# neofytr/LLMTokenizer

Measured on AMD Instinct MI355X. Metric: corpus MB/s per merge iter (train), 1 GiB synthetic corpus, higher is better.
Workload: dtype u32

## Files before the change

llmtokenizer_amd/csrc/batch.hip:

```cpp
#pragma once
#include "engine_common.h"

namespace bpeamd {

static_assert(TOPK == 64, "a wave holds a list, one entry per lane");
static_assert(BRB == 2 * (1024 / 64), "the select's 16 waves merge two partial lists each");
#ifndef BPE_SU
#define BPE_SU 1
#endif
#ifndef BPE_FORM_PRINT
#define BPE_FORM_PRINT 0
#endif
#ifndef BPE_RU
#define BPE_RU 4
#endif
#ifndef BPE_AU
#define BPE_AU 1
#endif
constexpr uint32_t AU = BPE_AU;
constexpr uint32_t SU = BPE_SU;
#ifndef BPE_RUN_THREAD_PAIRS
#define BPE_RUN_THREAD_PAIRS 16
#endif
constexpr uint32_t RUN_THREAD_PAIRS = BPE_RUN_THREAD_PAIRS, RUN_Q = 256;
#ifndef BPE_RUN_BLOCK_Q
#define BPE_RUN_BLOCK_Q 2
#endif
constexpr uint32_t RUN_BLOCK_Q = BPE_RUN_BLOCK_Q;
#ifndef BPE_RUN_BU
#define BPE_RUN_BU 2
#endif
constexpr uint32_t RUN_BU = BPE_RUN_BU;
#ifndef BPE_FR
#define BPE_FR (BPE_BK > 63 ? 3 : 4)
#endif
// ... 1048 lines not shown
            s = (s + 1) & (RH - 1);
        }
    }
    __device__ inline uint32_t member(uint32_t a, uint32_t b) const {
        const unsigned long long key = (((unsigned long long)a << 32) | b) + 1ull;
        uint32_t s = rp_hash(a, b);
        for (;;) {
            const unsigned long long v = pk[s];
            if (v == key) return pm[s];
            if (v == 0ull) return BK;
            s = (s + 1) & (RP - 1);
        }
    }
};

__device__ inline void vadd_b(uint32_t (*s)[DENSE], const Eng *E, uint32_t m, int v, uint32_t x, uint32_t *gcnt) {
    if (x < DENSE) {
        atomicAdd(&s[v][x], 1u);
        return;
    }
    const uint64_t base = ((uint64_t)m * 4 + v) * E->bvs;
    const uint32_t old = atomicAdd(&E->bvec[base + (x - DENSE)], 1u);
    if (old == 0) {
        const uint32_t p = atomicAdd(&E->bvnl[m * 4 + v], 1u);
        E->bvlist[base + p] = x;
    }
    if (v == V_DL || v == V_DR) atomicAdd(&gcnt[v], 1u);
}

__device__ inline void vadd_g(const Eng *E, uint32_t m, int v, uint32_t x, uint32_t cnt) {
    if (!cnt) return;
    if (x < DENSE) {
        atomicAdd(&E->bvecd[((uint64_t)m * BREPL * 4 + v) * DENSE + x], cnt);
        return;
    }
    const uint64_t base = ((uint64_t)m * 4 + v) * E->bvs;
    if (atomicAdd(&E->bvec[base + (x - DENSE)], cnt) == 0) {
        const uint32_t p = atomicAdd(&E->bvnl[m * 4 + v], 1u);
        E->bvlist[base + p] = x;
    }
}

__device__ inline void xadd(const Eng *E, uint32_t *xo, uint32_t Wx, uint32_t m, int v, uint32_t x) {
    if (x < Wx) {
        atomicAdd(&xo[2 + v * Wx + x], 1u);
        return;
    }
    const uint64_t base = ((uint64_t)m * 4 + v) * E->bvs;
    if (atomicAdd(&E->bvec[base + (x - DENSE)], 1u) == 0) {
        const uint32_t p = atomicAdd(&E->bvnl[m * 4 + v], 1u);
        E->bvlist[base + p] = x;
    }
}

struct BHalo {
    uint32_t HL[3], HR[3], hlr[BK], myi[BK];
};

template <bool SH>
__device__ inline uint32_t tok_at_b(const uint32_t *__restrict__ tok, const BHalo &H, int64_t p, int64_t n) {
    if (p < 0) return SH && p >= -3 ? get3(H.HL, (uint32_t)(-1 - p)) : HOLE;
    if (p >= n) return SH && p - n < 3 ? get3(H.HR, (uint32_t)(p - n)) : HOLE;
    return tok[p];
}

template <bool SH>
__device__ inline uint32_t cover_of(const uint32_t *__restrict__ tok, const RoleTab &rt, const BHalo &H, uint32_t p,
                                    int64_t ps, int64_t n) {
    if (!(rt.get(p) >> 31)) return BK;
    const int64_t pps = v_left<SH>(tok, ps);
    const uint32_t pp = tok_at_b<SH>(tok, H, pps, n);
    const uint32_t mm = rt.member(pp, p);
    if (mm >= BK || pp != p) return mm;
    uint32_t L;
    if (SH && ps < 0) {
        L = H.hlr[mm];
    } else {
        L = 1;
        int64_t x = v_left<SH>(tok, ps);
        for (; x >= 0 && tok[x] == p; x = v_left<SH>(tok, x)) L++;
        if (SH && x < 0) L += H.hlr[mm];
    }
    return (L & 1) ? BK : mm;
}

template <bool SH>
__device__ inline uint32_t starts_of(const uint32_t *__restrict__ tok, const RoleTab &rt, const BHalo &H, uint32_t q,
                                     int64_t kq, int64_t n) {
    const uint32_t lq = rt.get(q) & 0x7FFFFFFFu;
    if (!lq) return BK;
    const int64_t kn = v_right(kq, lq, n);
    return rt.member(q, tok_at_b<SH>(tok, H, kn, n));
}

enum : uint32_t { GRF_LGO = 1, GRF_LEND = 2, GRF_IGO = 3, GRF_IEND = 4 };
__device__ void bscan_long_runs(const Eng *__restrict__ E, Bat *__restrict__ B, const uint32_t *__restrict__ tok,
                                const RoleTab &rt, const BHalo &H, int64_t n, uint32_t z0, uint32_t sgen) {
    const uint32_t lane = threadIdx.x & 63;
    const uint32_t ng = uni(min(aload(&B->gr_n), GRUN));
    const uint64_t stride = gr_stride(E->n0), maxch = stride - 1;
    auto flag_of = [&](uint32_t st) { return (sgen << 3) | st; };
    for (uint32_t gi = 0; gi < ng; gi++) {
        uint32_t ok = 1;
        if (lane == 0) {
            const unsigned long long t0 = wall_clock64();
            while (__hip_atomic_load(&B->gr_ready[gi], __ATOMIC_ACQUIRE, __HIP_MEMORY_SCOPE_AGENT) != sgen) {
                if (wall_clock64() - t0 > E->gr_wait) {
                    ok = 0;
                    B->ra_err = 11;
                    atomicAdd(&B->gr_tready, 1u);
                    break;
// ... 135 lines not shown
                vadd_g(E, mg, V_DR, ag, nint_dr);
                vadd_g(E, mg, V_IR, zg, nint_ir);
                if (npairs) atomicAdd(&B->bound[mg], npairs);
                atomicAdd(&B->nchunks, 1ull);
            }
#pragma unroll
            for (uint32_t bb = 0; bb < NBK; bb++) {
                unsigned long long tm = tadj.w[bb];
                for (int o = 32; o > 0; o >>= 1) tm |= __shfl_xor(tm, o);
                if (lane == 0 && tm) atomicOr(&B->adj[mg][bb], tm);
            }
        }
    }
}

template <bool SH>
__global__ __launch_bounds__(SCAN_T) void k_bscan(const Eng *__restrict__ E, const Ctl *__restrict__ C) {
    if (C->stop) return;
    Bat *B = E->bat;
    const uint32_t bi = bat_idx(E);
    ts_mark(E, bi, BT_SCAN_IN, true);
    if (threadIdx.x == 0) atomicMax(&B->sc_in, ~wall_clock64());
    __shared__ uint32_t s[4][DENSE];
    __shared__ uint32_t list[SCAN_T * SU * FR];
    __shared__ uint16_t ltag[SCAN_T * SU * FR];
    __shared__ uint32_t lcount, gbase, list_n, covc, sm, sk, sz0, bRs;
    __shared__ uint32_t lr_n, lr_brk, lr_pos[RUN_Q];
    __shared__ unsigned long long badj[NBK];
    __shared__ uint32_t gcnt[2];
    __shared__ uint32_t sa[BK], sb[BK];
    __shared__ RoleTab rt;
    __shared__ BHalo H;
    __shared__ uint32_t wmx[2][16];
    const uint32_t tid = threadIdx.x;
    const uint32_t sgen = ((uint32_t)(B->nbatch + B->nretry) & 0x0FFFFFFFu) + 1u;
    if (tid == 0) {
        sm = BK;
        covc = lcount = bRs = 0;
// ... 41 lines not shown
    }
    const uint32_t a = sa[m], b = sb[m], z = z0 + m;
    const uint32_t la = E->tlen[a], lb = E->tlen[b];
    const uint32_t mode = B->mode[m], off = B->off[m], len = B->len[m];
    const uint32_t bid = blockIdx.x - B->blk0[m], nblk = B->blk0[m + 1] - B->blk0[m];
    const uint32_t sbase = B->sbase[m];
    uint32_t *occz = E->ids_out + sbase;
    uint16_t *tagz = E->btag + sbase;
    const uint32_t sslice = B->sbase[m + 1] - sbase;
#define STG(IDX, WHERE) if ((IDX) >= sslice) { B->ra_err = 12; } else
    uint32_t *Rm = &B->R[m];
    const int64_t n = (int64_t)E->n0;
    const uint32_t *__restrict__ tok = E->tok;
    const uint32_t want = mode == 2 ? a : b;
    const uint32_t lim = min(DENSE, z0 + k);
    for (uint32_t v = 0; v < 4; v++)
        for (uint32_t x = tid; x < lim; x += SCAN_T) s[v][x] = 0;
    __syncthreads();
    auto tok_at = [&](int64_t p) -> uint32_t { return tok_at_b<SH>(tok, H, p, n); };

    if (a != b) {
        static_assert(SU == 1 && BPE_WFLUSH, "the wave-driven candidate loop: one entry per lane per round");
        const uint32_t stride = nblk * SCAN_T;
        const uint32_t lane = tid & 63, wbase = (tid >> 6) * 64 * FR;
        uint32_t wcnt = 0, wocc = 0;
        uint32_t nent[SU];
        uint16_t ntg[SU];
        uint32_t eS = bid * SCAN_T + (tid & ~63u);
        auto load1 = [&](uint32_t s0, uint32_t &en, uint16_t &tg) {
            const uint32_t e = s0 + lane;
            en = 0;
            tg = 0xFFFFu;
            if (e < len) {
                en = mode == 0 ? E->plist[off + e] : E->occ[off + e];
                if (mode) tg = E->occnb[off + e];
            }
        };
        uint32_t pent = 0;
        uint16_t ptg = 0xFFFFu;
        auto advance = [&]() {
            eS += stride;
            if (SCAN_PD > 1) {
                nent[0] = pent;
                ntg[0] = ptg;
                if (eS + stride < len) load1(eS + stride, pent, ptg);
            } else if (eS < len) {
                load1(eS, nent[0], ntg[0]);
            }
        };
        auto flush = [&]() {
            __builtin_amdgcn_fence(__ATOMIC_RELEASE, "wavefront");
            __builtin_amdgcn_wave_barrier();
            uint32_t g = 0;
            if (lane == 0 && wcnt) g = atomicAdd(Rm, wcnt);
            g = __shfl(g, 0);
            for (uint32_t q = lane; q < wcnt; q += 64) {
                STG(g + q, "wflush") {
                occz[g + q] = list[wbase + q];
                tagz[g + q] = ltag[wbase + q];
                }
            }
            wocc += wcnt;
            wcnt = 0;
            __builtin_amdgcn_wave_barrier();
        };
        const bool cmp = mode != 0 && E->scan_compact != 0;
        const uint32_t tsh = mode == 2 ? 8u : 0u;
        uint32_t qpos = 0, qn = 0;
        load1(eS, nent[0], ntg[0]);
        if (SCAN_PD > 1) load1(eS + stride, pent, ptg);
        for (;;) {
            uint32_t ent[SU];
            uint16_t etg[SU];
            bool val[SU];
            if (!cmp) {
                if (eS >= len) break;
                val[0] = eS + lane < len;
                ent[0] = nent[0];
                etg[0] = ntg[0];
                advance();
            } else {
                while (eS < len) {
                    const bool pass = eS + lane < len && tag_ok(((uint32_t)ntg[0] >> tsh) & 0xFFu, want);
                    const unsigned long long M = __ballot(pass);
                    const uint32_t np = (uint32_t)__popcll(M);
                    if (qn + np > 64) break;
                    const uint32_t r = lane - qn;
                    const bool mine = lane >= qn && r < np;
                    const uint32_t pv = (uint32_t)__shfl((int)nent[0], (int)(mine ? kth_bit(M, r) : lane));
                    if (mine) qpos = pv;
                    qn += np;
                    advance();
                }
                if (qn == 0) break;
                val[0] = lane < qn;
                ent[0] = qpos;
                etg[0] = 0xFFFFu;
                qn = 0;
            }
            int64_t ii[SU], jj[SU];
            TokWin W[SU];
#pragma unroll
            for (uint32_t u = 0; u < SU; u++) {
                if (mode == 2) {
                    val[u] = val[u] && tag_ok(etg[u] >> 8, want);
                    jj[u] = ent[u];
                    ii[u] = 0;
                    if (val[u]) W[u] = tok_window(tok, jj[u]);
                } else {
                    val[u] = val[u] && (mode == 0 || tag_ok(etg[u] & 0xFFu, want));
                    ii[u] = ent[u];
                    jj[u] = ii[u] + la;
                    if (val[u]) W[u] = tok_window(tok, ii[u]);
                }
            }
            bool ok[SU];
            uint32_t tl[SU], tr[SU];
#pragma unroll
            for (uint32_t u = 0; u < SU; u++) {
                ok[u] = false;
                tl[u] = tr[u] = HOLE;
                if (!val[u]) continue;
                const int64_t j = jj[u];
                if (mode == 2) {
                    const uint32_t wl = j > 0 ? W[u].at(j - 1) : HOLE;
                    const int64_t i = j > 0 ? start_of_end<SH>(wl, j - 1) : -1;
                    ii[u] = i;
                    if (W[u].at(j) != b || i < 0) continue;
                    const uint32_t ti = W[u].has(i) ? W[u].at(i) : tok[i];
                    tl[u] = i > 0 ? (W[u].has(i - 1) ? W[u].at(i - 1) : tok[i - 1]) : HOLE;
                    const int64_t kk = j + lb;
                    tr[u] = kk < n ? (W[u].has(kk) ? W[u].at(kk) : tok[kk]) : HOLE;
                    ok[u] = ti == a;
                } else {
                    const int64_t i = ii[u], kk = j + lb;
                    const uint32_t t1 = j >= n ? HOLE : W[u].has(j) ? W[u].at(j) : tok[j];
                    tl[u] = i > 0 ? W[u].at(i - 1) : HOLE;
                    tr[u] = kk >= n ? HOLE : W[u].has(kk) ? W[u].at(kk) : tok[kk];
                    ok[u] = W[u].at(i) == a && t1 == b && j < n;
                }
            }
            int64_t ps[SU];
            uint32_t pv[SU];
#pragma unroll
            for (uint32_t u = 0; u < SU; u++) {
                const int64_t i = ii[u];
                ps[u] = i <= 0 ? -1 : start_of_end<SH>(tl[u], i - 1);
                pv[u] = ok[u] ? ((i > 0 && is_id(tl[u])) ? tl[u] : tok_at(ps[u])) : HOLE;
            }
#pragma unroll
            for (uint32_t u = 0; u < SU; u++) {
                const int64_t i = ii[u], j = jj[u];
                uint32_t lfin = HOLE, rfin = HOLE;
                if (ok[u]) {
                    const uint32_t p = pv[u];
                    lfin = p;
                    if (p != HOLE) {
                        const uint32_t cv = cover_of<SH>(tok, rt, H, p, ps[u], n);
                        if (cv < BK) {
                            lfin = z0 + cv;
                            mk_set(tadj, cv);
                            atomicAdd(&covc, 1u);
                        } else {
                            vadd_b(s, E, m, V_DL, p, gcnt);
                            vadd_b(s, E, m, V_IL, p, gcnt);
                        }
                    }
                    const int64_t kq = v_right(j, lb, n);
                    const uint32_t q = kq < n ? tr[u] : tok_at(kq);
                    rfin = q;
                    if (q != HOLE) {
                        const uint32_t st = starts_of<SH>(tok, rt, H, q, kq, n);
                        if (st < BK) {
                            rfin = z0 + st;
                            mk_set(tadj, st);
                        }
                        vadd_b(s, E, m, V_DR, q, gcnt);
                        vadd_b(s, E, m, V_IR, rfin, gcnt);
                    }
                }
                const unsigned long long om = __ballot(ok[u]);
                if (ok[u]) {
                    const uint32_t slot = wbase + wcnt + (uint32_t)__popcll(om & ((1ull << lane) - 1ull));
                    list[slot] = (uint32_t)i;
                    ltag[slot] = nb_tag(lfin, rfin);
                }
                wcnt += (uint32_t)__popcll(om);
            }
            if (wcnt + 64 > 64 * FR) flush();
        }
        if (wcnt) flush();
        if (lane == 0 && wocc) atomicAdd(&bRs, wocc);
    } else {
        for (uint32_t e0 = bid * SCAN_T; e0 < len; e0 += nblk * SCAN_T) {
            const uint32_t e = e0 + tid;
            int64_t i = 0;
            bool ok = false;
            if (e >= len) {
            } else if (mode == 2) {
                const int64_t j = E->occ[off + e];
                if (tag_ok(E->occnb[off + e] >> 8, want) && tok[j] == b) {
                    i = v_left<SH>(tok, j);
                    ok = i >= 0 && tok[i] == a;
                }
// ... 23 lines not shown
                const uint32_t rq = nocc ? z : st < BK ? z0 + st : q;
                if (st < BK) mk_set(tadj, st);
                const uint32_t pfin = (mi > 0 || cont) ? z : (left ? p : cv < BK ? z0 + cv : HOLE);
                const uint32_t slot = atomicAdd(&lcount, 1u);
                if (slot < SCAN_T * SU) {
                    list[slot] = (uint32_t)pos;
                    ltag[slot] = nb_tag(pfin, rq);
                } else {
                    const uint32_t g = atomicAdd(Rm, 1u);
                    atomicAdd(&bRs, 1u);
                    STG(g, "tstraight") {
                    occz[g] = (uint32_t)pos;
                    tagz[g] = nb_tag(pfin, rq);
                    }
                }
                if (mi == 0 && left) {
                    vadd_b(s, E, m, V_DL, p, gcnt);
                    vadd_b(s, E, m, V_IL, p, gcnt);
                }
                if (q != HOLE) {
                    vadd_b(s, E, m, V_DR, q, gcnt);
                    vadd_b(s, E, m, V_IR, rq, gcnt);
                }
                if (!knext || kq >= n) break;
                if (mi + 1 >= RUN_THREAD_PAIRS && nocc) {
                    if (!SH && E->grflag && kq + (int64_t)GR_PROBE * la < n && tok[kq + (int64_t)GR_PROBE * la] == a) {
                        const uint32_t gi = atomicAdd(&B->gr_n, 1u);
                        if (gi < GRUN) {
                            B->gr_c[gi] = (uint32_t)kq;
                            B->gr_m[gi] = m;
                            atomicAdd(&B->gr_nreg, 1u);
                            __hip_atomic_store(&B->gr_ready[gi], sgen, __ATOMIC_RELEASE, __HIP_MEMORY_SCOPE_AGENT);
                            break;
                        }
// ... 104 lines not shown
                    });
                    const bool done = lr_brk < NS;
                    __syncthreads();
                    if (done) break;
                    c += (int64_t)NS * 64 * la;
                }
            }
        }
    }
    __syncthreads();
    if (!SH && E->grflag) bscan_long_runs(E, B, tok, rt, H, n, z0, sgen);
    ts_mark(E, bi, BT_SCAN_CAND, false, true);
    if (tid < SKMAX && tid < B->nsk && ((B->sk_cm[tid][m >> 6] >> (m & 63)) & 1ull)) {
        const uint32_t xs = B->sk_a[tid], ys = B->sk_b[tid];
        uint32_t d = 0;
        if (xs == b && ys < lim) d += s[V_DR][ys];
        if (ys == a && xs < lim) d += s[V_DL][xs];
        if (d) atomicAdd(SH ? &E->xbat[BK + tid] : &B->sdec[tid], d);
    }
    const uint32_t Wx = xbat_vw(z0 + k);
    uint32_t *xm = SH ? E->xbat + XBH + (uint64_t)m * xbat_member_words(Wx) : nullptr;
    if (SH && blockIdx.x == 0 && tid == 0) {
        uint32_t xlm = BK;
        const int64_t F1 = C->F1, L1 = C->L1;
        const uint32_t over = B->over;
        if (F1 < n) {
            const uint32_t tf = tok[F1], tl1 = tok[L1];
            for (uint32_t mm = 0; mm < k; mm++)
                if (H.HL[0] == sa[mm] && tf == sb[mm] && (sa[mm] != sb[mm] || (H.hlr[mm] & 1))) {
                    xlm = mm;
                    break;
                }
// ... 37 lines not shown
    if (k > 1) {
#pragma unroll
        for (uint32_t bb = 0; bb < NBK; bb++) {
            unsigned long long t = tadj.w[bb];
            for (int o = 32; o > 0; o >>= 1) t |= __shfl_xor(t, o);
            if ((tid & 63) == 0 && t) atomicOr(&badj[bb], t);
        }
        __syncthreads();
        if (tid < NBK && badj[tid]) atomicOr(&B->adj[m][tid], badj[tid]);
    }
    uint32_t *rep = SH ? xm + 2 : E->bvecd + (uint64_t)(m * BREPL + bid % BREPL) * 4 * DENSE;
    const uint32_t vstride = SH ? Wx : DENSE;
    uint32_t mxl = 0, mxr = 0;
    for (uint32_t v = 0; v < 4; v++)
        for (uint32_t x = tid; x < lim; x += SCAN_T) {
            const uint32_t c = s[v][x];
            if (c) atomicAdd(&rep[v * vstride + x], c);
            if (v == V_DL) mxl = max(mxl, c);
            if (v == V_DR) mxr = max(mxr, c);
        }
    if (SH && tid == 0 && bRs) atomicAdd(&xm[0], bRs);
    if (k > 1) {
        for (int o = 32; o > 0; o >>= 1) {
            mxl = max(mxl, (uint32_t)__shfl_xor(mxl, o));
            mxr = max(mxr, (uint32_t)__shfl_xor(mxr, o));
        }
        if ((tid & 63) == 0) {
            wmx[0][tid >> 6] = mxl;
            wmx[1][tid >> 6] = mxr;
        }
        __syncthreads();
        if (tid == 0) {
            uint32_t l = 0, r = 0;
            for (uint32_t q = 0; q < SCAN_T / 64; q++) {
                l = max(l, wmx[0][q]);
                r = max(r, wmx[1][q]);
            }
            atomicAdd(SH ? &xm[1] : &B->bound[m], max(l + gcnt[V_DL] + covc, r + gcnt[V_DR]));
        }
    }
    ts_mark(E, bi, BT_SCAN_OUT, false, true);
    asm volatile("s_waitcnt vmcnt(0)" ::: "memory");
    __syncthreads();
    if (tid == 0) atomicMax(&B->sc_out, wall_clock64());
}
template __global__ void k_bscan<false>(const Eng *, const Ctl *);
template __global__ void k_bscan<true>(const Eng *, const Ctl *);

constexpr uint32_t XSP_SHIFT = 23;
static_assert(4 * BK < (1u << (32 - XSP_SHIFT)), "member-vector index fits above the id");
__global__ __launch_bounds__(256) void k_bpack(const Eng *__restrict__ E, const Ctl *__restrict__ C) {
    if (C->stop) return;
    const Bat *B = E->bat;
    __shared__ uint32_t pre[BK * 4 + 1];
    __shared__ uint32_t written;
    const uint32_t k = B->k, tid = threadIdx.x, nmv = 4 * k;
    if (tid < 64) {
        constexpr uint32_t LP = 4 * NBK;
        uint32_t c[LP], sum = 0;
#pragma unroll
        for (uint32_t j = 0; j < LP; j++) {
            c[j] = LP * tid + j < nmv ? E->bvnl[LP * tid + j] : 0u;
// ... 652 lines not shown
```

llmtokenizer_amd/csrc/engine.hip:

```cpp
#include <hip/hip_runtime.h>
#include <fcntl.h>
#include <unistd.h>
#include <cerrno>

#include <algorithm>
#include <chrono>
#include <cstdio>
#include <cstdlib>
#include <cstring>
#include <string>
#include <thread>
#include <vector>
#include <unordered_map>

#include <rocprim/rocprim.hpp>

#include "../../include/bpe_gpu.h"
#include "kernels.hip"
#include "batch.hip"
#include "encode.hip"
#include "encode_win.hip"
#include "encode_docs.hip"
#include "split.hip"
#include "train_split.hip"
// ... 529 lines not shown
        if ((r = dalloc(c, &h.hotp_best, SPEC_RB))) return r;
        if ((r = dalloc(c, &h.hotp_key, SPEC_RB))) return r;
        if ((r = dalloc(c, &h.hotp_v2, SPEC_RB))) return r;
        if ((r = dalloc(c, &h.hotp_k2, SPEC_RB))) return r;
        if ((r = dalloc(c, &h.hotp_tie, SPEC_RB))) return r;
    }
    h.batch = getenv_int("BPE_BATCH", 1) && h.hot && h.vcap <= BATCH_VCAP_MAX && (!c->sharded || c->sbatch) &&
                      (c->sharded || c->fast || n0 >= TRACK_LIMIT)
                  ? 1
                  : 0;
    h.skip_on = (uint32_t)(getenv_int("BPE_SKIP", 1) != 0);
    if (h.skip_on && getenv_int("BPE_SKIP_TEST", 0)) h.skip_on = 2;
    h.skg_exp = (uint32_t)getenv_int("BPE_SKGATE", 2);
    h.scan_occd = (uint32_t)std::max(0, getenv_int("BPE_SCAN_OCCD", 6));
    h.scan_compact = (uint32_t)(getenv_int("BPE_SCAN_COMPACT", 1) != 0);
    {
        int nl = BK > 63 ? 2 : 1;
        if (getenv_int("BPE_LIST2", 0)) nl = std::max(nl, 2);
        nl = getenv_int("BPE_NLIST", nl);
        h.nlists = (uint32_t)std::max(1, std::min(nl, (int)NLIST));
    }
    h.tie_up = (uint32_t)(getenv_int("BPE_TIE_UP", 0) != 0);
    h.crate_pct = (uint32_t)std::max(100, getenv_int("BPE_CRATE_PCT", 200));
    h.lose_retry = (uint32_t)(getenv_int("BPE_TEST_LOSE_RETRY", 0) != 0);
    h.xbat = nullptr;
    h.xsp_out = h.xsp_in = nullptr;
    h.xsp_cap = 0;
    h.xsp_stride = 0;
    h.bat = nullptr;
    h.btag = nullptr;
// ... 216 lines not shown
        }
        return 0;
    }
    k_hot_collect<<<slots ? std::max<uint32_t>(1, std::min<uint32_t>(256, (ns + 255) / 256)) : 2048, 256, 0, c->st>>>(
        c->dE, c->dC, slots, ns);
    HIPCHK(hipGetLastError());
    return 0;
}

void launch_argmax_inputs(bpe_gpu_ctx *c) {
    launch_summaries(c);
    if (c->h.hot) k_hot_reduce<<<c->h.hot_parts, 1024, 0, c->st>>>(c->dE, c->dC);
}

void launch_batch(bpe_gpu_ctx *c) {
    k_bscan<false><<<BSB, SCAN_T, 0, c->st>>>(c->dE, c->dC);
    k_bapply<false><<<BAPPLY_B + BAPPLY_RA, 1024, 0, c->st>>>(c->dE, c->dC, BAPPLY_B);
    k_bsel<<<BRB + BAPPLY_A, 1024, 0, c->st>>>(c->dE, c->dC);
}

bool fused_graph(const bpe_gpu_ctx *c, bool tracked) { return c->h.spec_on && (!tracked || c->h.track_ub == 1); }

void launch_iteration(bpe_gpu_ctx *c, bool tracked) {
    if (fused_graph(c, tracked)) {
        const uint32_t trk = c->h.track_ub == 1 && !c->fast && c->n0 < TRACK_LIMIT ? 1 + (c->h.lcap ? LIGHT_B : 0) : 0;
        k_rescan_spec<<<SPEC_RB + SPEC_SB + trk, SCAN_T, 0, c->st>>>(c->dE, c->dC, SPEC_RB, trk);
        if (c->h.hcap / L1W > SELECT_L1_MAX && !c->h.hot) k_rescan2<<<RESCAN2_BLOCKS, 256, 0, c->st>>>(c->dE, c->dC);
        k_fused<<<1 + FUSED_A + FUSED_B, 1024, 0, c->st>>>(c->dE, c->dC, FUSED_A, nullptr);
        return;
    }
    k_scan<false><<<tracked ? TSCAN_BLOCKS : SCAN_BLOCKS, SCAN_T, 0, c->st>>>(c->dE, c->dC);
// ... 2840 lines not shown
```

llmtokenizer_amd/csrc/engine_common.h:

```cpp
#pragma once
#include <hip/hip_runtime.h>
#include <stddef.h>
#include <stdint.h>

namespace bpeamd {

constexpr uint32_t HOLE = 0xFFFFFFFFu;
constexpr uint32_t END_FLAG = 0x80000000u;
constexpr uint32_t MARKV = 0xFFFFFFFEu;
constexpr uint64_t END_MAX = 0x7FFFFFFDull;
__host__ __device__ inline bool is_id(uint32_t v) { return v < END_FLAG; }
__host__ __device__ inline uint32_t end_code(uint64_t d) { return END_FLAG | (uint32_t)d; }
#ifndef BPE_DENSE
#define BPE_DENSE 8192
#endif
constexpr uint32_t DENSE = BPE_DENSE;
#ifndef BPE_REPL
#define BPE_REPL 8
#endif
constexpr uint32_t REPL = BPE_REPL;
constexpr uint32_t NTHR = 16;
constexpr uint64_t CHUNK = 65536;
constexpr uint64_t DYN_LIMIT = CHUNK * NTHR;
constexpr uint64_t TRACK_LIMIT = 2 * DYN_LIMIT;
// ... 199 lines not shown
    uint32_t *erec;
    const uint32_t *enc_pairs;
    uint32_t n_enc;
    EncBatch *eb;
    uint32_t hot;
    uint32_t hot_parts;
    uint32_t hot_target;
    uint32_t relist_stale;
    uint32_t *hot_slot;
    uint32_t *hot_hist;
    unsigned long long *hotp_best, *hotp_key, *hotp_v2, *hotp_k2;
    uint32_t *hotp_tie;
    uint32_t batch;
    uint32_t skip_on;
    uint32_t scan_compact;
    uint32_t scan_occd;
    uint32_t skg_exp;
    uint32_t nlists;
    uint32_t tie_up;
    uint32_t crate_pct;
    uint32_t lose_retry;
    uint32_t bvs;
    Bat *bat;
    uint16_t *btag;
    uint32_t *bvecd;
    uint32_t *bvec;
    uint32_t *bvlist;
    uint32_t *bvnl;
    uint32_t *xbat;
    uint32_t *grflag;
// ... 203 lines not shown
```

llmtokenizer_amd/csrc/kernels.hip:

```cpp
#include "engine_common.h"
#include "p2p.hip"

namespace bpeamd {

__device__ inline uint32_t lane_id() { return __lane_id(); }

__device__ inline uint32_t aload(const uint32_t *p) {
    return __hip_atomic_load(p, __ATOMIC_RELAXED, __HIP_MEMORY_SCOPE_AGENT);
}
__device__ inline void astore(uint32_t *p, uint32_t v) {
    __hip_atomic_store(p, v, __ATOMIC_RELAXED, __HIP_MEMORY_SCOPE_AGENT);
}
__device__ inline unsigned long long aload64(const unsigned long long *p) {
    return __hip_atomic_load(p, __ATOMIC_RELAXED, __HIP_MEMORY_SCOPE_AGENT);
}

__device__ inline uint32_t wave_append(bool pred, uint32_t *counter) {
    unsigned long long m = __ballot(pred);
    if (m == 0) return 0;
    uint32_t lane = lane_id();
    uint32_t leader = __ffsll(m) - 1;
    uint32_t base = 0;
    if (lane == leader) base = atomicAdd(counter, (uint32_t)__popcll(m));
    base = __shfl(base, leader);
// ... 67 lines not shown
__device__ inline uint32_t id_at(const uint32_t *__restrict__ tok, HaloT &h, int64_t p, int64_t n) {
    if (p < 0) return SH && p >= -3 ? get3(h.get().HL, (uint32_t)(-1 - p)) : HOLE;
    if (p >= n) return SH && p - n < 3 ? get3(h.get().HR, (uint32_t)(p - n)) : HOLE;
    return tok[p];
}

template <bool SH = true>
__device__ inline int64_t start_of_end(uint32_t v, int64_t e) {
    if (is_id(v)) return e;
    if (SH && v == MARKV) return -1;
    const int64_t d = v & ~END_FLAG;
    if (!SH) return e - d;
    return d > e ? -1 : e - d;
}

template <bool SH = true>
__device__ inline int64_t v_left(const uint32_t *__restrict__ tok, int64_t p) {
    if (p <= 0) return p - 1;
    return start_of_end<SH>(tok[p - 1], p - 1);
}

__device__ inline int64_t v_right(int64_t p, uint32_t len, int64_t n) {
    if (p >= n) return p + 1;
    const int64_t q = p + len;
    return q >= n ? n : q;
}

constexpr uint32_t SCAN_T = 1024;

struct TokWin {
    uint4 w0, w1;
    int64_t base;
    __device__ inline bool has(int64_t x) const { return x >= base && x < base + 8; }
    __device__ inline uint32_t at(int64_t x) const {
        const uint32_t k = (uint32_t)(x - base);
        const uint4 w = k < 4 ? w0 : w1;
        const uint32_t r = k & 3;
        return r == 0 ? w.x : r == 1 ? w.y : r == 2 ? w.z : w.w;
    }
};

__device__ inline TokWin tok_window(const uint32_t *__restrict__ tok, int64_t i) {
    TokWin W;
    W.base = (i > 0 ? i - 1 : 0) & ~3ll;
    const uint4 *p = reinterpret_cast<const uint4 *>(tok + W.base);
    W.w0 = p[0];
    W.w1 = p[1];
    return W;
}

__device__ inline uint16_t nb_tag(uint32_t p, uint32_t q) {
    const uint32_t p8 = p == HOLE ? 0xFFu : (p & 0xFFu), q8 = q == HOLE ? 0xFFu : (q & 0xFFu);
    return (uint16_t)((p8 << 8) | q8);
}
__device__ inline bool tag_ok(uint32_t t8, uint32_t id) { return t8 == 0xFFu || t8 == (id & 0xFFu); }

__device__ inline void flush_list(uint32_t *list, uint16_t *ltag, uint32_t *lcount, uint32_t *gbase, uint32_t *R,
                                  uint32_t *occz, uint16_t *tagz, uint32_t *bcount) {
    __syncthreads();
    const uint32_t n = min(*lcount, SCAN_T);
    if (threadIdx.x == 0) {
        *gbase = n ? atomicAdd(R, n) : 0;
// ... 3185 lines not shown
```

llmtokenizer_amd/csrc/shard.hip:

```cpp
#include <dlfcn.h>
#include <rccl/rccl.h>


namespace {

struct RcclApi {
    void *lib = nullptr;
    ncclResult_t (*getUniqueId)(ncclUniqueId *) = nullptr;
    ncclResult_t (*commInitRank)(ncclComm_t *, int, ncclUniqueId, int) = nullptr;
    ncclResult_t (*allReduce)(const void *, void *, size_t, ncclDataType_t, ncclRedOp_t, ncclComm_t,
                              hipStream_t) = nullptr;
    ncclResult_t (*allGather)(const void *, void *, size_t, ncclDataType_t, ncclComm_t, hipStream_t) = nullptr;
    ncclResult_t (*commDestroy)(ncclComm_t) = nullptr;
    const char *(*errStr)(ncclResult_t) = nullptr;
};

int rccl_api(RcclApi **out) {
    static RcclApi api;
    if (!api.lib) {
        void *l = dlopen("librccl.so.1", RTLD_NOW | RTLD_GLOBAL);
        if (!l) l = dlopen("/opt/rocm/lib/librccl.so.1", RTLD_NOW | RTLD_GLOBAL);
        if (!l) return fail(BPE_GPU_ENODEV, "librccl.so.1 not loadable");
        api.getUniqueId = (decltype(api.getUniqueId))dlsym(l, "ncclGetUniqueId");
        api.commInitRank = (decltype(api.commInitRank))dlsym(l, "ncclCommInitRank");
// ... 192 lines not shown
    }
    if (g->rccl) {
        ncclResult_t e = g->rccl->allGather(c0->h.xsp_out, c0->h.xsp_in, stride, ncclUint32, g->comm, g->st);
        if (e != ncclSuccess) return rccl_fail(g->rccl, "ncclAllGather", e);
        return 0;
    }
    const uint32_t K = (uint32_t)g->cs.size();
    k_xspgather<<<K * K * 8, 256, 0, g->st>>>(g->d_ptrs + 4 * K, g->d_ptrs + 5 * K, K, stride);
    HIPCHK(hipGetLastError());
    return 0;
}

int launch_group_bstep(bpe_gpu_group *g) {
    int r;
    const bool sparse = g->cs[0]->h.xsp_out != nullptr;
    for (bpe_gpu_ctx *c : g->cs) k_bscan<true><<<BSB, SCAN_T, 0, g->st>>>(c->dE, c->dC);
    if (sparse)
        for (bpe_gpu_ctx *c : g->cs) k_bpack<<<64, 256, 0, g->st>>>(c->dE, c->dC);
    if ((r = ex_bsum(g))) return r;
    if (sparse && (r = ex_sparse(g))) return r;
    for (bpe_gpu_ctx *c : g->cs) k_bapply<true><<<BAPPLY_B + BAPPLY_RA, 1024, 0, g->st>>>(c->dE, c->dC, BAPPLY_B);
    for (bpe_gpu_ctx *c : g->cs) k_bsel<<<BRB + BAPPLY_A, 1024, 0, g->st>>>(c->dE, c->dC);
    HIPCHK(hipGetLastError());
    return ex_records(g, g->d_ptrs);
}

int group_bselect(bpe_gpu_group *g) {
    for (bpe_gpu_ctx *c : g->cs) k_bsel<<<BRB + BAPPLY_A, 1024, 0, g->st>>>(c->dE, c->dC);
    for (bpe_gpu_ctx *c : g->cs) k_edges<<<1, 256, 0, g->st>>>(c->dE, c->dC, 1);
    HIPCHK(hipGetLastError());
    return ex_records(g, g->d_ptrs);
// ... 997 lines not shown
```

Baseline: 114.9 million.

## Restructure bscan candidate loop to hoist dependent token loads and shrink shared histograms

Reworks the scan kernel's candidate loop so the dependent global token fetches (window, fringe tokens, left/right neighbour lookups, role-table flags) are issued in separate batched phases before use. The aim is more memory-level parallelism and fewer serialized load chains. Pointers are cast to the global address space so the compiler can emit plain global loads, and the shared histogram shrinks from four rows to three because the DL and IL rows are merged. An optional two-candidates-per-lane variant is added behind an env knob, but it is off by default. The cost is higher register pressure and some speculative loads for inactive lanes.

```diff
diff --git a/llmtokenizer_amd/csrc/batch.hip b/llmtokenizer_amd/csrc/batch.hip
--- a/llmtokenizer_amd/csrc/batch.hip
+++ b/llmtokenizer_amd/csrc/batch.hip
@@ -5,9 +5,6 @@
 
 static_assert(TOPK == 64, "a wave holds a list, one entry per lane");
 static_assert(BRB == 2 * (1024 / 64), "the select's 16 waves merge two partial lists each");
-#ifndef BPE_SU
-#define BPE_SU 1
-#endif
 #ifndef BPE_FORM_PRINT
 #define BPE_FORM_PRINT 0
 #endif
@@ -18,7 +15,6 @@
 #define BPE_AU 1
 #endif
 constexpr uint32_t AU = BPE_AU;
-constexpr uint32_t SU = BPE_SU;
 #ifndef BPE_RUN_THREAD_PAIRS
 #define BPE_RUN_THREAD_PAIRS 16
 #endif
@@ -1097,11 +1093,10 @@
     }
 };
 
-__device__ inline void vadd_b(uint32_t (*s)[DENSE], const Eng *E, uint32_t m, int v, uint32_t x, uint32_t *gcnt) {
-    if (x < DENSE) {
-        atomicAdd(&s[v][x], 1u);
-        return;
-    }
+enum { S_L = 0, S_DR = 1, S_IR = 2, S_N = 3 };
+__device__ constexpr int s_row(int v) { return v == V_DR ? S_DR : v == V_IR ? S_IR : S_L; }
+
+__device__ inline void vadd_bg(const Eng *E, uint32_t m, int v, uint32_t x, uint32_t *gcnt) {
     const uint64_t base = ((uint64_t)m * 4 + v) * E->bvs;
     const uint32_t old = atomicAdd(&E->bvec[base + (x - DENSE)], 1u);
     if (old == 0) {
@@ -1111,6 +1106,23 @@
     if (v == V_DL || v == V_DR) atomicAdd(&gcnt[v], 1u);
 }
 
+__device__ inline void vadd_b(uint32_t (*s)[DENSE], const Eng *E, uint32_t m, int v, uint32_t x, uint32_t *gcnt) {
+    if (x < DENSE) {
+        atomicAdd(&s[s_row(v)][x], 1u);
+        return;
+    }
+    vadd_bg(E, m, v, x, gcnt);
+}
+
+__device__ inline void vadd_bl(uint32_t (*s)[DENSE], const Eng *E, uint32_t m, uint32_t x, uint32_t *gcnt) {
+    if (x < DENSE) {
+        atomicAdd(&s[S_L][x], 1u);
+        return;
+    }
+    vadd_bg(E, m, V_DL, x, gcnt);
+    vadd_bg(E, m, V_IL, x, gcnt);
+}
+
 __device__ inline void vadd_g(const Eng *E, uint32_t m, int v, uint32_t x, uint32_t cnt) {
     if (!cnt) return;
     if (x < DENSE) {
@@ -1140,21 +1152,15 @@
     uint32_t HL[3], HR[3], hlr[BK], myi[BK];
 };
 
-template <bool SH>
-__device__ inline uint32_t tok_at_b(const uint32_t *__restrict__ tok, const BHalo &H, int64_t p, int64_t n) {
+template <bool SH, typename TP>
+__device__ inline uint32_t tok_at_b(TP tok, const BHalo &H, int64_t p, int64_t n) {
     if (p < 0) return SH && p >= -3 ? get3(H.HL, (uint32_t)(-1 - p)) : HOLE;
     if (p >= n) return SH && p - n < 3 ? get3(H.HR, (uint32_t)(p - n)) : HOLE;
     return tok[p];
 }
 
-template <bool SH>
-__device__ inline uint32_t cover_of(const uint32_t *__restrict__ tok, const RoleTab &rt, const BHalo &H, uint32_t p,
-                                    int64_t ps, int64_t n) {
-    if (!(rt.get(p) >> 31)) return BK;
-    const int64_t pps = v_left<SH>(tok, ps);
-    const uint32_t pp = tok_at_b<SH>(tok, H, pps, n);
-    const uint32_t mm = rt.member(pp, p);
-    if (mm >= BK || pp != p) return mm;
+template <bool SH, typename TP>
+__device__ inline bool run_odd(TP tok, const BHalo &H, uint32_t p, int64_t ps, uint32_t mm) {
     uint32_t L;
     if (SH && ps < 0) {
         L = H.hlr[mm];
@@ -1164,12 +1170,21 @@
         for (; x >= 0 && tok[x] == p; x = v_left<SH>(tok, x)) L++;
         if (SH && x < 0) L += H.hlr[mm];
     }
-    return (L & 1) ? BK : mm;
-}
-
-template <bool SH>
-__device__ inline uint32_t starts_of(const uint32_t *__restrict__ tok, const RoleTab &rt, const BHalo &H, uint32_t q,
-                                     int64_t kq, int64_t n) {
+    return L & 1;
+}
+
+template <bool SH, typename TP>
+__device__ inline uint32_t cover_of(TP tok, const RoleTab &rt, const BHalo &H, uint32_t p, int64_t ps, int64_t n) {
+    if (!(rt.get(p) >> 31)) return BK;
+    const int64_t pps = v_left<SH>(tok, ps);
+    const uint32_t pp = tok_at_b<SH>(tok, H, pps, n);
+    const uint32_t mm = rt.member(pp, p);
+    if (mm >= BK || pp != p) return mm;
+    return run_odd<SH>(tok, H, p, ps, mm) ? BK : mm;
+}
+
+template <bool SH, typename TP>
+__device__ inline uint32_t starts_of(TP tok, const RoleTab &rt, const BHalo &H, uint32_t q, int64_t kq, int64_t n) {
     const uint32_t lq = rt.get(q) & 0x7FFFFFFFu;
     if (!lq) return BK;
     const int64_t kn = v_right(kq, lq, n);
@@ -1177,7 +1192,7 @@
 }
 
 enum : uint32_t { GRF_LGO = 1, GRF_LEND = 2, GRF_IGO = 3, GRF_IEND = 4 };
-__device__ void bscan_long_runs(const Eng *__restrict__ E, Bat *__restrict__ B, const uint32_t *__restrict__ tok,
+__device__ __attribute__((always_inline)) inline void bscan_long_runs(const Eng *__restrict__ E, Bat *__restrict__ B, const uint32_t *__restrict__ tok,
                                 const RoleTab &rt, const BHalo &H, int64_t n, uint32_t z0, uint32_t sgen) {
     const uint32_t lane = threadIdx.x & 63;
     const uint32_t ng = uni(min(aload(&B->gr_n), GRUN));
@@ -1343,14 +1358,15 @@
     }
 }
 
-template <bool SH>
+template <bool SH, uint32_t SU>
 __global__ __launch_bounds__(SCAN_T) void k_bscan(const Eng *__restrict__ E, const Ctl *__restrict__ C) {
+    static_assert(SU == 1 || SU == 2, "one or two candidates per lane");
     if (C->stop) return;
     Bat *B = E->bat;
     const uint32_t bi = bat_idx(E);
     ts_mark(E, bi, BT_SCAN_IN, true);
     if (threadIdx.x == 0) atomicMax(&B->sc_in, ~wall_clock64());
-    __shared__ uint32_t s[4][DENSE];
+    __shared__ uint32_t s[S_N][DENSE];
     __shared__ uint32_t list[SCAN_T * SU * FR];
     __shared__ uint16_t ltag[SCAN_T * SU * FR];
     __shared__ uint32_t lcount, gbase, list_n, covc, sm, sk, sz0, bRs;
@@ -1422,38 +1438,52 @@
     const uint32_t *__restrict__ tok = E->tok;
     const uint32_t want = mode == 2 ? a : b;
     const uint32_t lim = min(DENSE, z0 + k);
-    for (uint32_t v = 0; v < 4; v++)
+    for (uint32_t v = 0; v < S_N; v++)
         for (uint32_t x = tid; x < lim; x += SCAN_T) s[v][x] = 0;
     __syncthreads();
     auto tok_at = [&](int64_t p) -> uint32_t { return tok_at_b<SH>(tok, H, p, n); };
 
     if (a != b) {
-        static_assert(SU == 1 && BPE_WFLUSH, "the wave-driven candidate loop: one entry per lane per round");
-        const uint32_t stride = nblk * SCAN_T;
-        const uint32_t lane = tid & 63, wbase = (tid >> 6) * 64 * FR;
+        static_assert(BPE_WFLUSH, "the wave-driven candidate loop stages per wave");
+        const uint32_t *const tokf = tok;
+        const auto tok = as_global(tokf);
+        const auto occz = as_global(E->ids_out) + sbase;
+        const auto tagz = as_global(E->btag) + sbase;
+        auto tok_at = [&](int64_t p) -> uint32_t { return tok_at_b<SH>(tok, H, p, n); };
+        constexpr uint32_t SEG = 64 * SU;
+        const uint32_t stride = nblk * SCAN_T * SU;
+        const uint32_t lane = tid & 63, wbase = (tid >> 6) * SEG * FR;
         uint32_t wcnt = 0, wocc = 0;
         uint32_t nent[SU];
         uint16_t ntg[SU];
-        uint32_t eS = bid * SCAN_T + (tid & ~63u);
-        auto load1 = [&](uint32_t s0, uint32_t &en, uint16_t &tg) {
-            const uint32_t e = s0 + lane;
-            en = 0;
-            tg = 0xFFFFu;
-            if (e < len) {
-                en = mode == 0 ? E->plist[off + e] : E->occ[off + e];
-                if (mode) tg = E->occnb[off + e];
+        uint32_t eS = (bid * SCAN_T + (tid & ~63u)) * SU;
+        const auto lst = as_global((const uint32_t *)(mode == 0 ? E->plist : E->occ)) + off;
+        const auto lnb = as_global((const uint16_t *)E->occnb) + off;
+        auto load1 = [&](uint32_t s0, uint32_t (&en)[SU], uint16_t (&tg)[SU]) {
+#pragma unroll
+            for (uint32_t u = 0; u < SU; u++) {
+                const uint32_t e = s0 + 64 * u + lane;
+                en[u] = 0;
+                tg[u] = 0xFFFFu;
+                if (e < len) {
+                    en[u] = lst[e];
+                    if (mode) tg[u] = lnb[e];
+                }
             }
         };
-        uint32_t pent = 0;
-        uint16_t ptg = 0xFFFFu;
+        uint32_t pent[SU];
+        uint16_t ptg[SU];
         auto advance = [&]() {
             eS += stride;
             if (SCAN_PD > 1) {
-                nent[0] = pent;
-                ntg[0] = ptg;
+#pragma unroll
+                for (uint32_t u = 0; u < SU; u++) {
+                    nent[u] = pent[u];
+                    ntg[u] = ptg[u];
+                }
                 if (eS + stride < len) load1(eS + stride, pent, ptg);
             } else if (eS < len) {
-                load1(eS, nent[0], ntg[0]);
+                load1(eS, nent, ntg);
             }
         };
         auto flush = [&]() {
@@ -1474,8 +1504,10 @@
         };
         const bool cmp = mode != 0 && E->scan_compact != 0;
         const uint32_t tsh = mode == 2 ? 8u : 0u;
-        uint32_t qpos = 0, qn = 0;
-        load1(eS, nent[0], ntg[0]);
+        uint32_t qpos[SU], qn = 0;
+#pragma unroll
+        for (uint32_t u = 0; u < SU; u++) qpos[u] = 0;
+        load1(eS, nent, ntg);
         if (SCAN_PD > 1) load1(eS + stride, pent, ptg);
         for (;;) {
             uint32_t ent[SU];
@@ -1483,27 +1515,45 @@
             bool val[SU];
             if (!cmp) {
                 if (eS >= len) break;
-                val[0] = eS + lane < len;
-                ent[0] = nent[0];
-                etg[0] = ntg[0];
+#pragma unroll
+                for (uint32_t u = 0; u < SU; u++) {
+                    val[u] = eS + 64 * u + lane < len;
+                    ent[u] = nent[u];
+                    etg[u] = ntg[u];
+                }
                 advance();
             } else {
                 while (eS < len) {
-                    const bool pass = eS + lane < len && tag_ok(((uint32_t)ntg[0] >> tsh) & 0xFFu, want);
-                    const unsigned long long M = __ballot(pass);
-                    const uint32_t np = (uint32_t)__popcll(M);
-                    if (qn + np > 64) break;
-                    const uint32_t r = lane - qn;
-                    const bool mine = lane >= qn && r < np;
-                    const uint32_t pv = (uint32_t)__shfl((int)nent[0], (int)(mine ? kth_bit(M, r) : lane));
-                    if (mine) qpos = pv;
-                    qn += np;
+                    unsigned long long M[SU];
+                    uint32_t np = 0;
+#pragma unroll
+                    for (uint32_t u = 0; u < SU; u++) {
+                        M[u] = __ballot(eS + 64 * u + lane < len && tag_ok(((uint32_t)ntg[u] >> tsh) & 0xFFu, want));
+                        np += (uint32_t)__popcll(M[u]);
+                    }
+                    if (qn + np > SEG) break;
+#pragma unroll
+                    for (uint32_t u = 0; u < SU; u++) {
+                        const uint32_t npu = (uint32_t)__popcll(M[u]);
+#pragma unroll
+                        for (uint32_t v = 0; v < SU; v++) {
+                            if (qn + npu <= 64 * v || qn >= 64 * (v + 1)) continue;
+                            const uint32_t r = 64 * v + lane - qn;
+                            const bool mine = 64 * v + lane >= qn && r < npu;
+                            const uint32_t pv = (uint32_t)__shfl((int)nent[u], (int)(mine ? kth_bit(M[u], r) : lane));
+                            if (mine) qpos[v] = pv;
+                        }
+                        qn += npu;
+                    }
                     advance();
                 }
                 if (qn == 0) break;
-                val[0] = lane < qn;
-                ent[0] = qpos;
-                etg[0] = 0xFFFFu;
+#pragma unroll
+                for (uint32_t u = 0; u < SU; u++) {
+                    val[u] = 64 * u + lane < qn;
+                    ent[u] = qpos[u];
+                    etg[u] = 0xFFFFu;
+                }
                 qn = 0;
             }
             int64_t ii[SU], jj[SU];
@@ -1514,13 +1564,32 @@
                     val[u] = val[u] && tag_ok(etg[u] >> 8, want);
                     jj[u] = ent[u];
                     ii[u] = 0;
-                    if (val[u]) W[u] = tok_window(tok, jj[u]);
                 } else {
                     val[u] = val[u] && (mode == 0 || tag_ok(etg[u] & 0xFFu, want));
                     ii[u] = ent[u];
                     jj[u] = ii[u] + la;
-                    if (val[u]) W[u] = tok_window(tok, ii[u]);
-                }
+                }
+            }
+#pragma unroll
+            for (uint32_t u = 0; u < SU; u++) W[u] = tok_window(tok, val[u] ? (mode == 2 ? jj[u] : ii[u]) : 0);
+            bool live[SU];
+            uint32_t f1[SU], fl[SU], fr[SU];
+#pragma unroll
+            for (uint32_t u = 0; u < SU; u++) {
+                live[u] = val[u];
+                f1[u] = fl[u] = fr[u] = HOLE;
+                const int64_t j = jj[u], kk = j + lb;
+                if (mode == 2) {
+                    const uint32_t wl = val[u] && j > 0 ? W[u].at(j - 1) : HOLE;
+                    const int64_t i = val[u] && j > 0 ? start_of_end<SH>(wl, j - 1) : -1;
+                    ii[u] = i;
+                    live[u] = val[u] && i >= 0 && W[u].at(j) == b;
+                    if (live[u] && !W[u].has(i)) f1[u] = tok[i];
+                    if (live[u] && i > 0 && !W[u].has(i - 1)) fl[u] = tok[i - 1];
+                } else {
+                    if (live[u] && j < n && !W[u].has(j)) f1[u] = tok[j];
+                }
+                if (live[u] && kk < n && !W[u].has(kk)) fr[u] = tok[kk];
             }
             bool ok[SU];
             uint32_t tl[SU], tr[SU];
@@ -1528,23 +1597,17 @@
             for (uint32_t u = 0; u < SU; u++) {
                 ok[u] = false;
                 tl[u] = tr[u] = HOLE;
-                if (!val[u]) continue;
-                const int64_t j = jj[u];
+                if (!live[u]) continue;
+                const int64_t i = ii[u], j = jj[u], kk = j + lb;
                 if (mode == 2) {
-                    const uint32_t wl = j > 0 ? W[u].at(j - 1) : HOLE;
-                    const int64_t i = j > 0 ? start_of_end<SH>(wl, j - 1) : -1;
-                    ii[u] = i;
-                    if (W[u].at(j) != b || i < 0) continue;
-                    const uint32_t ti = W[u].has(i) ? W[u].at(i) : tok[i];
-                    tl[u] = i > 0 ? (W[u].has(i - 1) ? W[u].at(i - 1) : tok[i - 1]) : HOLE;
-                    const int64_t kk = j + lb;
-                    tr[u] = kk < n ? (W[u].has(kk) ? W[u].at(kk) : tok[kk]) : HOLE;
+                    const uint32_t ti = W[u].has(i) ? W[u].at(i) : f1[u];
+                    tl[u] = i > 0 ? (W[u].has(i - 1) ? W[u].at(i - 1) : fl[u]) : HOLE;
+                    tr[u] = kk < n ? (W[u].has(kk) ? W[u].at(kk) : fr[u]) : HOLE;
                     ok[u] = ti == a;
                 } else {
-                    const int64_t i = ii[u], kk = j + lb;
-                    const uint32_t t1 = j >= n ? HOLE : W[u].has(j) ? W[u].at(j) : tok[j];
+                    const uint32_t t1 = j >= n ? HOLE : W[u].has(j) ? W[u].at(j) : f1[u];
                     tl[u] = i > 0 ? W[u].at(i - 1) : HOLE;
-                    tr[u] = kk >= n ? HOLE : W[u].has(kk) ? W[u].at(kk) : tok[kk];
+                    tr[u] = kk >= n ? HOLE : W[u].has(kk) ? W[u].at(kk) : fr[u];
                     ok[u] = W[u].at(i) == a && t1 == b && j < n;
                 }
             }
@@ -1556,29 +1619,49 @@
                 ps[u] = i <= 0 ? -1 : start_of_end<SH>(tl[u], i - 1);
                 pv[u] = ok[u] ? ((i > 0 && is_id(tl[u])) ? tl[u] : tok_at(ps[u])) : HOLE;
             }
+            uint32_t qv[SU], pfl[SU], qfl[SU];
+            int64_t kq[SU];
 #pragma unroll
             for (uint32_t u = 0; u < SU; u++) {
-                const int64_t i = ii[u], j = jj[u];
+                kq[u] = v_right(jj[u], lb, n);
+                qv[u] = ok[u] ? (kq[u] < n ? tr[u] : tok_at(kq[u])) : HOLE;
+                pfl[u] = pv[u] != HOLE ? rt.get(pv[u]) >> 31 : 0u;
+                qfl[u] = qv[u] != HOLE ? rt.get(qv[u]) & 0x7FFFFFFFu : 0u;
+            }
+            uint32_t cw[SU], sw[SU];
+#pragma unroll
+            for (uint32_t u = 0; u < SU; u++) {
+                cw[u] = sw[u] = HOLE;
+                if (pfl[u] && ps[u] > 0) cw[u] = tok[ps[u] - 1];
+                if (qfl[u]) sw[u] = tok_at(v_right(kq[u], qfl[u], n));
+            }
+            uint32_t pp[SU];
+#pragma unroll
+            for (uint32_t u = 0; u < SU; u++) {
+                pp[u] = HOLE;
+                if (pfl[u]) pp[u] = tok_at(ps[u] <= 0 ? ps[u] - 1 : start_of_end<SH>(cw[u], ps[u] - 1));
+            }
+#pragma unroll
+            for (uint32_t u = 0; u < SU; u++) {
                 uint32_t lfin = HOLE, rfin = HOLE;
                 if (ok[u]) {
                     const uint32_t p = pv[u];
                     lfin = p;
                     if (p != HOLE) {
-                        const uint32_t cv = cover_of<SH>(tok, rt, H, p, ps[u], n);
+                        uint32_t cv = pfl[u] ? rt.member(pp[u], p) : BK;
+                        if (cv < BK && pp[u] == p && run_odd<SH>(tok, H, p, ps[u], cv)) cv = BK;
                         if (cv < BK) {
                             lfin = z0 + cv;
                             mk_set(tadj, cv);
                             atomicAdd(&covc, 1u);
                         } else {
-                            vadd_b(s, E, m, V_DL, p, gcnt);
-                            vadd_b(s, E, m, V_IL, p, gcnt);
+                            vadd_bl(s, E, m, p, gcnt);
                         }
                     }
-                    const int64_t kq = v_right(j, lb, n);
-                    const uint32_t q = kq < n ? tr[u] : tok_at(kq);
+                    const uint32_t q = qv[u];
                     rfin = q;
                     if (q != HOLE) {
-                        const uint32_t st = starts_of<SH>(tok, rt, H, q, kq, n);
+                        const uint32_t st = qfl[u] ? rt.member(q, sw[u]) : BK;
                         if (st < BK) {
                             rfin = z0 + st;
                             mk_set(tadj, st);
@@ -1590,12 +1673,12 @@
                 const unsigned long long om = __ballot(ok[u]);
                 if (ok[u]) {
                     const uint32_t slot = wbase + wcnt + (uint32_t)__popcll(om & ((1ull << lane) - 1ull));
-                    list[slot] = (uint32_t)i;
+                    list[slot] = (uint32_t)ii[u];
                     ltag[slot] = nb_tag(lfin, rfin);
                 }
                 wcnt += (uint32_t)__popcll(om);
             }
-            if (wcnt + 64 > 64 * FR) flush();
+            if (wcnt + SEG > SEG * FR) flush();
         }
         if (wcnt) flush();
         if (lane == 0 && wocc) atomicAdd(&bRs, wocc);
@@ -1649,10 +1732,7 @@
                     tagz[g] = nb_tag(pfin, rq);
                     }
                 }
-                if (mi == 0 && left) {
-                    vadd_b(s, E, m, V_DL, p, gcnt);
-                    vadd_b(s, E, m, V_IL, p, gcnt);
-                }
+                if (mi == 0 && left) vadd_bl(s, E, m, p, gcnt);
                 if (q != HOLE) {
                     vadd_b(s, E, m, V_DR, q, gcnt);
                     vadd_b(s, E, m, V_IR, rq, gcnt);
@@ -1787,8 +1867,8 @@
     if (tid < SKMAX && tid < B->nsk && ((B->sk_cm[tid][m >> 6] >> (m & 63)) & 1ull)) {
         const uint32_t xs = B->sk_a[tid], ys = B->sk_b[tid];
         uint32_t d = 0;
-        if (xs == b && ys < lim) d += s[V_DR][ys];
-        if (ys == a && xs < lim) d += s[V_DL][xs];
+        if (xs == b && ys < lim) d += s[S_DR][ys];
+        if (ys == a && xs < lim) d += s[S_L][xs];
         if (d) atomicAdd(SH ? &E->xbat[BK + tid] : &B->sdec[tid], d);
     }
     const uint32_t Wx = xbat_vw(z0 + k);
@@ -1856,7 +1936,7 @@
     uint32_t mxl = 0, mxr = 0;
     for (uint32_t v = 0; v < 4; v++)
         for (uint32_t x = tid; x < lim; x += SCAN_T) {
-            const uint32_t c = s[v][x];
+            const uint32_t c = s[s_row(v)][x];
             if (c) atomicAdd(&rep[v * vstride + x], c);
             if (v == V_DL) mxl = max(mxl, c);
             if (v == V_DR) mxr = max(mxr, c);
@@ -1886,8 +1966,11 @@
     __syncthreads();
     if (tid == 0) atomicMax(&B->sc_out, wall_clock64());
 }
-template __global__ void k_bscan<false>(const Eng *, const Ctl *);
-template __global__ void k_bscan<true>(const Eng *, const Ctl *);
+template <bool SH>
+inline void launch_bscan(const Eng *dE, const Ctl *dC, uint32_t su, hipStream_t st) {
+    if (su == 2) k_bscan<SH, 2><<<BSB, SCAN_T, 0, st>>>(dE, dC);
+    else k_bscan<SH, 1><<<BSB, SCAN_T, 0, st>>>(dE, dC);
+}
 
 constexpr uint32_t XSP_SHIFT = 23;
 static_assert(4 * BK < (1u << (32 - XSP_SHIFT)), "member-vector index fits above the id");
diff --git a/llmtokenizer_amd/csrc/engine.hip b/llmtokenizer_amd/csrc/engine.hip
--- a/llmtokenizer_amd/csrc/engine.hip
+++ b/llmtokenizer_amd/csrc/engine.hip
@@ -567,6 +567,7 @@
     h.skg_exp = (uint32_t)getenv_int("BPE_SKGATE", 2);
     h.scan_occd = (uint32_t)std::max(0, getenv_int("BPE_SCAN_OCCD", 6));
     h.scan_compact = (uint32_t)(getenv_int("BPE_SCAN_COMPACT", 1) != 0);
+    h.scan_su = getenv_int("BPE_SCAN_SU", 1) == 2 ? 2u : 1u;
     {
         int nl = BK > 63 ? 2 : 1;
         if (getenv_int("BPE_LIST2", 0)) nl = std::max(nl, 2);
@@ -813,7 +814,7 @@
 }
 
 void launch_batch(bpe_gpu_ctx *c) {
-    k_bscan<false><<<BSB, SCAN_T, 0, c->st>>>(c->dE, c->dC);
+    launch_bscan<false>(c->dE, c->dC, c->h.scan_su, c->st);
     k_bapply<false><<<BAPPLY_B + BAPPLY_RA, 1024, 0, c->st>>>(c->dE, c->dC, BAPPLY_B);
     k_bsel<<<BRB + BAPPLY_A, 1024, 0, c->st>>>(c->dE, c->dC);
 }
diff --git a/llmtokenizer_amd/csrc/engine_common.h b/llmtokenizer_amd/csrc/engine_common.h
--- a/llmtokenizer_amd/csrc/engine_common.h
+++ b/llmtokenizer_amd/csrc/engine_common.h
@@ -237,6 +237,7 @@
     uint32_t batch;
     uint32_t skip_on;
     uint32_t scan_compact;
+    uint32_t scan_su;
     uint32_t scan_occd;
     uint32_t skg_exp;
     uint32_t nlists;
diff --git a/llmtokenizer_amd/csrc/kernels.hip b/llmtokenizer_amd/csrc/kernels.hip
--- a/llmtokenizer_amd/csrc/kernels.hip
+++ b/llmtokenizer_amd/csrc/kernels.hip
@@ -4,6 +4,15 @@
 namespace bpeamd {
 
 __device__ inline uint32_t lane_id() { return __lane_id(); }
+
+#define BPE_GLOBAL __attribute__((address_space(1)))
+template <typename T>
+__device__ __attribute__((always_inline)) inline T BPE_GLOBAL *as_global(T *p) {
+    return (T BPE_GLOBAL *)p;
+}
+typedef uint32_t u32x4_t __attribute__((ext_vector_type(4)));
+__device__ inline u32x4_t load_x4(const uint32_t *p) { return *reinterpret_cast<const u32x4_t *>(p); }
+__device__ inline u32x4_t load_x4(const uint32_t BPE_GLOBAL *p) { return *(const u32x4_t BPE_GLOBAL *)p; }
 
 __device__ inline uint32_t aload(const uint32_t *p) {
     return __hip_atomic_load(p, __ATOMIC_RELAXED, __HIP_MEMORY_SCOPE_AGENT);
@@ -105,8 +114,8 @@
     return d > e ? -1 : e - d;
 }
 
-template <bool SH = true>
-__device__ inline int64_t v_left(const uint32_t *__restrict__ tok, int64_t p) {
+template <bool SH = true, typename TP = const uint32_t *>
+__device__ inline int64_t v_left(TP tok, int64_t p) {
     if (p <= 0) return p - 1;
     return start_of_end<SH>(tok[p - 1], p - 1);
 }
@@ -131,12 +140,13 @@
     }
 };
 
-__device__ inline TokWin tok_window(const uint32_t *__restrict__ tok, int64_t i) {
+template <typename TP>
+__device__ inline TokWin tok_window(TP tok, int64_t i) {
     TokWin W;
     W.base = (i > 0 ? i - 1 : 0) & ~3ll;
-    const uint4 *p = reinterpret_cast<const uint4 *>(tok + W.base);
-    W.w0 = p[0];
-    W.w1 = p[1];
+    const u32x4_t a = load_x4(tok + W.base), b = load_x4(tok + W.base + 4);
+    W.w0 = make_uint4(a.x, a.y, a.z, a.w);
+    W.w1 = make_uint4(b.x, b.y, b.z, b.w);
     return W;
 }
 
diff --git a/llmtokenizer_amd/csrc/shard.hip b/llmtokenizer_amd/csrc/shard.hip
--- a/llmtokenizer_amd/csrc/shard.hip
+++ b/llmtokenizer_amd/csrc/shard.hip
@@ -230,7 +230,7 @@
 int launch_group_bstep(bpe_gpu_group *g) {
     int r;
     const bool sparse = g->cs[0]->h.xsp_out != nullptr;
-    for (bpe_gpu_ctx *c : g->cs) k_bscan<true><<<BSB, SCAN_T, 0, g->st>>>(c->dE, c->dC);
+    for (bpe_gpu_ctx *c : g->cs) launch_bscan<true>(c->dE, c->dC, c->h.scan_su, g->st);
     if (sparse)
         for (bpe_gpu_ctx *c : g->cs) k_bpack<<<64, 256, 0, g->st>>>(c->dE, c->dC);
     if ((r = ex_bsum(g))) return r;
```

Result: no change. 115.8 million, median of 6 (+0.7%).
